# leodd/Lifted-Hybrid-Variational-Inference

Hardware: AMD Instinct MI355X
Metric: lbp_sweeps_per_sec_10M_edge_hybrid_mrf (higher is better)
Workload: dtype f64

## Files before the change

include/lhvi.h:

```cpp
#ifndef LHVI_H
#define LHVI_H

#include <stddef.h>
#include <stdint.h>

#ifdef __cplusplus
extern "C" {
#endif

#define LHVI_ABI_VERSION 19
#define LHVI_MAX_ARITY 6

#define LHVI_OK 0
#define LHVI_E_ARG (-1)
#define LHVI_E_LAUNCH (-2)
#define LHVI_E_UNSUPPORTED (-3)
#define LHVI_E_NODEVICE (-4)
#define LHVI_E_NOT_PD (-5)

#define LHVI_POT_GENERIC 0
#define LHVI_POT_TABLE 1
#define LHVI_POT_GAUSSIAN 2
#define LHVI_POT_QUADRATIC 3
#define LHVI_POT_HYBRID_QUADRATIC 4
#define LHVI_POT_LINEAR_GAUSSIAN 5
#define LHVI_POT_X2 6
#define LHVI_POT_XY 7
#define LHVI_POT_MLN 8
#define LHVI_POT_MLN_HARD 9
#define LHVI_POT_IMAGE_NODE 10
#define LHVI_POT_IMAGE_EDGE 11

typedef struct lhvi_graph {
// ... 68 lines not shown
int lhvi_log_likelihood(const lhvi_graph_t* g, const lhvi_pots_t* pots, const double* x, double* out, void* ws, size_t ws_bytes,
                        void* stream);


#define LHVI_PBP_EP 1u
#define LHVI_PBP_EPBP_DISCRETE 2u
#define LHVI_PBP_SKIP_TERMS 16u
#define LHVI_PBP_LEAVE_ROOM 256u
#define LHVI_PBP_CQ 512u
#define LHVI_PBP_BOUNDARY_TOTALS 2048u
#define LHVI_PBP_NO_UNIQ 4096u
#define LHVI_PBP_V2F_RECORDS 8192u
#define LHVI_PBP_WIDE_PAIRS 16384u
#define LHVI_PBP_SHARE_CUS 32768u
#define LHVI_PBP_NO_GRID 128u
#define LHVI_PBP_FUSED_RECORDS16 131072u
#define LHVI_PBP_F2V_HEAVY 262144u
#define LHVI_PBP_F2V_SMALL 524288u
#define LHVI_PBP_F2V_PAIR 1048576u
#define LHVI_PBP_F2V_FAST 2097152u
#define LHVI_PBP_F2V_CQ 4194304u
#define LHVI_PBP_F2V_GENERIC 8388608u
#define LHVI_PBP_F2V_ALL (LHVI_PBP_F2V_HEAVY | LHVI_PBP_F2V_SMALL | LHVI_PBP_F2V_PAIR | LHVI_PBP_F2V_FAST | LHVI_PBP_F2V_CQ | LHVI_PBP_F2V_GENERIC)
#define LHVI_PBP_POW2_GROUPS 65536u

typedef struct lhvi_pbp {
    int32_t n;
    int32_t T;
    uint32_t flags;
    double var_threshold;
    double max_log_value;
    const double* particles;
    const double* old_particles;
    const int32_t* np;
    const uint8_t* uniq;
    const double* q;
    const int32_t* fast_edges;
    int32_t n_fast;
    const int32_t* generic_edges;
    int32_t n_generic;
    int32_t generic_pts_log2;
    const void* fast_desc;
    const void* heavy_desc;
    int32_t n_heavy;
    const void* light_desc;
    int32_t n_light;
// ... 13 lines not shown
    const void* cq_desc;
    int32_t n_cq;
    const int32_t* v2f_wide;
    int32_t n_v2f_wide;
    const int32_t* v2f_narrow;
    int32_t n_v2f_narrow;
    const int32_t* v2f_hub;
    int32_t n_v2f_hub;
    const int32_t* v2f_mid16;
    int32_t n_v2f_mid16;
    const int32_t* v2f_mid32;
    int32_t n_v2f_mid32;
    const int32_t* prop_hub;
    int32_t n_prop_hub;
    double* prop_partial;
    const int32_t* resample_vars;
    int32_t n_resample_vars;
    const void* small16_desc;
    int32_t n_small16;
    const void* small32_desc;
    int32_t n_small32;
    const int64_t* halo_off;
    double* halo_buf;
} lhvi_pbp_t;

#define LHVI_PBP_DESC_BYTES 128
#define LHVI_PBP_TICKET_WORDS 16
#define LHVI_PBP_TICKET_COUNTERS 8
int lhvi_pbp_describe(const lhvi_graph_t* g, const lhvi_pots_t* pots, const lhvi_pbp_t* s, const int32_t* edges, int32_t count,
                      void* desc_out, void* stream);
int lhvi_pbp_describe_cq(const lhvi_graph_t* g, const lhvi_pots_t* pots, const lhvi_pbp_t* s, const int32_t* edges, int32_t count,
                         void* desc_out, void* stream);
int lhvi_pbp_var_sum(const lhvi_graph_t* g, const lhvi_pbp_t* s, const double* f2v, double* out, void* stream);
int lhvi_pbp_domain_grid(const lhvi_graph_t* g, const lhvi_pbp_t* s, double* x, void* stream);
int lhvi_pbp_refine_grid(const lhvi_graph_t* g, const lhvi_pbp_t* s, const double* logb, double* x, double* best, double* best_val,
                         void* stream);
int lhvi_debug_exp(const double* x, double* y, int64_t n, void* stream);
int lhvi_debug_exp_acc(const double* x, const double* c, double* y, int64_t n, void* stream);
int lhvi_debug_exp_acc_floor(const double* x, const double* c, double* y, int64_t n, void* stream);
int lhvi_debug_log(const double* x, double* y, int64_t n, int32_t which, void* stream);

int lhvi_pbp_classify(const lhvi_graph_t* g, const lhvi_pots_t* pots, const lhvi_pbp_t* s, uint8_t* edge_class, void* stream);

int lhvi_pbp_uniq(const lhvi_graph_t* g, int32_t n, const double* particles, const int32_t* np, uint8_t* uniq, void* stream);
int lhvi_pbp_v2f(const lhvi_graph_t* g, const lhvi_pbp_t* s, const double* f2v, double* v2f, void* stream);
int lhvi_pbp_f2v(const lhvi_graph_t* g, const lhvi_pots_t* pots, const lhvi_pbp_t* s, const double* v2f, double* f2v, void* stream);
int lhvi_pbp_proposal(const lhvi_graph_t* g, const lhvi_pbp_t* s, const double* f2v, double* eta, double* q, void* stream);
int lhvi_pbp_proposal_partial(const lhvi_graph_t* g, const lhvi_pbp_t* s, const double* f2v, double* eta, double* ph, void* stream);
int lhvi_pbp_proposal_finish(const lhvi_graph_t* g, const lhvi_pbp_t* s, const double* ph, double* q, void* stream);
int lhvi_pbp_boundary_pack(const lhvi_graph_t* g, const lhvi_pbp_t* s, const double* f2v, const double* ph, int32_t nb,
                           const int32_t* bvars, double* send, void* stream);
int lhvi_pbp_boundary_reduce(int32_t n_items, const int32_t* width, const int32_t* src_ptr, const int64_t* src_off,
                             const int32_t* dst_ptr, const int64_t* dst_off, const double* in, double* out, void* stream);
int lhvi_pbp_init(const lhvi_graph_t* g, const lhvi_pbp_t* s, double* eta, double* q, double* f2v, double* v2f, void* stream);
int lhvi_pbp_resample(const lhvi_graph_t* g, const lhvi_pbp_t* s, const int64_t* var_gid, uint64_t seed, uint32_t iteration, double* particles_out, void* stream);
int lhvi_pbp_edge_points(const lhvi_graph_t* g, const lhvi_pots_t* pots, const lhvi_pbp_t* s, const double* v2f,
                         int32_t nq, const int32_t* qedge, int32_t npts, const double* x, double* out, void* stream);
int lhvi_pbp_resample_uniq(const lhvi_graph_t* g, const lhvi_pbp_t* s, const int64_t* var_gid, uint64_t seed, uint32_t iteration,
                           double* particles_out, uint8_t* uniq_out, void* stream);
int lhvi_pbp_belief_points(const lhvi_graph_t* g, const lhvi_pots_t* pots, const lhvi_pbp_t* s, const double* v2f,
                           int32_t nq, const int32_t* qvar, int32_t npts, const double* x, double* out, void* stream);
int lhvi_pbp_var_fused(const lhvi_graph_t* g, const lhvi_pbp_t* s, const double* f2v, double* v2f, double* eta, double* q,
                       const int64_t* var_gid, uint64_t seed, uint32_t iteration, double* particles_out, uint8_t* uniq_out,
                       const int32_t* desc, int32_t n16, int32_t n32_t32, int32_t n32_t64, void* stream);
int lhvi_pbp_quad(const lhvi_graph_t* g, const lhvi_pots_t* pots, const lhvi_pbp_t* s, const double* v2f, int64_t nq,
                  const int32_t* row_var, const int64_t* qptr, const int32_t* qedge, const double* qmult, const double* lo,
                  const double* hi, double epsabs, double epsrel, double* z, double* abserr, int32_t* status, void* stream);
int lhvi_pbp_map_brent(const lhvi_graph_t* g, const lhvi_pots_t* pots, const lhvi_pbp_t* s, const double* v2f, int64_t nq,
// ... 235 lines not shown
```

lifted-hybrid-variational-inference_amd/csrc/pbp.hip:

```cpp
#include "common.hpp"
#include "potential.hpp"
#include "fastmath.hpp"
#include "cq.hpp"

namespace lhvi {

__device__ __forceinline__ double wave_sum(double v) { return dpp_wave_reduce(v, SumOp()); }
__device__ __forceinline__ double wave_max(double v) { return dpp_wave_reduce(v, MaxOp()); }
__device__ __forceinline__ int wave_sum_i(int v) {
#pragma unroll
    for (int off = 32; off > 0; off >>= 1) v += __shfl_xor(v, off);
    return v;
}

constexpr double PAD_LOG_TERM = -6.0e5;

__host__ __device__ __forceinline__ int var_first(const lhvi_pbp_t& s) { return s.var_hi > s.var_lo ? s.var_lo : 0; }
__host__ __device__ __forceinline__ int var_limit(const lhvi_graph_t& g, const lhvi_pbp_t& s) { return s.var_hi > s.var_lo ? s.var_hi : g.V; }

__device__ __forceinline__ double norm_pdf_std(double x, double mu, double sig) {
    const double u = (x - mu) / sig;
    return exp(-u * u * 0.5) / (2.506628274631 * sig);
}

__device__ __forceinline__ double log_importance(const lhvi_graph_t& g, const lhvi_pbp_t& s, int v, int d, double x,
                                                 double mu, double rsd , double log_norm) {
    const double LOG_1E200 = 460.51701859880916;
    if (g.dom_cont[d]) {
        if (x == g.dom_lo[d] || x == g.dom_hi[d]) return -LOG_1E200;
    } else {
        if (!(s.flags & LHVI_PBP_EPBP_DISCRETE)) return 0.0;
        const int b = g.dom_ptr[d];
        const int ns = g.dom_ptr[d + 1] - b;
        if (x == g.dom_val[b] || (ns > 1 && x == g.dom_val[b + 1])) return -LOG_1E200;
    }
    const double u = (x - mu) * rsd;
    return fmin(u * u * 0.5 + log_norm, LOG_1E200);
}

__global__ void __launch_bounds__(BLOCK) pbp_uniq_kernel(int V, int n, const double* __restrict__ particles,
                                                        const int32_t* __restrict__ np, uint8_t* __restrict__ uniq) {
    const int64_t i = (int64_t)blockIdx.x * BLOCK + threadIdx.x;
    if (i >= (int64_t)V * n) return;
    const int v = (int)(i / n), j = (int)(i % n);
    int u = j < np[v];
    const double x = particles[i];
    const double* row = particles + (int64_t)v * n;
    for (int k = 0; k < j && u; ++k)
// ... 884 lines not shown
    auto p = (const __attribute__((address_space(4))) char*)__builtin_amdgcn_kernarg_segment_ptr();
    asm volatile("" : "+s"(p));
    return *(const __attribute__((address_space(4))) T*)(p + offset);
}
struct HeavyHead {
    int32_t e, tv, pv, pce, cls, pos, kind, nj, np, T, gb, par_off;
    double pval;
    int32_t type, grid;
};
struct HeavyCoef { double ay, by, c, axy, bx, kx, gx0, gh; };
struct HeavyDesc { HeavyHead h; HeavyCoef k; };
static_assert(sizeof(HeavyDesc) == sizeof(FastDesc) && offsetof(HeavyDesc, k) == offsetof(FastDesc, ay) &&
              offsetof(HeavyHead, pval) == offsetof(FastDesc, pval) && offsetof(HeavyHead, grid) == offsetof(FastDesc, pad) + 4 &&
              offsetof(HeavyCoef, gx0) + offsetof(HeavyDesc, k) == offsetof(FastDesc, pad2), "HeavyDesc is FastDesc in two halves");

template <typename T> using global_ptr = __attribute__((address_space(1))) T*;
template <typename T>
__device__ __forceinline__ global_ptr<T> scalar_row(T* p) { global_ptr<T> q = (global_ptr<T>)p; asm("" : "+s"(q)); return q; }

template <typename T>
__device__ __forceinline__ T row_load(global_ptr<T> row, uint32_t i) { return *(global_ptr<T>)((global_ptr<const char>)row + i * (uint32_t)sizeof(T)); }
template <typename T>
__device__ __forceinline__ void row_store(global_ptr<T> row, uint32_t i, T v) { *(global_ptr<T>)((global_ptr<char>)row + i * (uint32_t)sizeof(T)) = v; }

__device__ __forceinline__ HeavyData heavy_fetch(const HeavyHead& d, const HeavyArgs& s, const double* __restrict__ v2f, int lane) {
    HeavyData h;
    const int n = s.n, np = d.np, npts = grid_eligible(d.grid, d.nj, d.T) ? d.np : d.np + d.T;
    const uint32_t ul = (uint32_t)lane;
    const auto prow = scalar_row(s.particles + (int64_t)d.tv * n);
    const auto grid_row = [&] { return scalar_row(heavy_arg_reload<const double*>(offsetof(HeavyArgs, dom_val)) + d.gb); };
    h.y = d.pval; h.m = 0.0; h.x0 = 0.0; h.x1 = 0.0;
    if (is_hidden(d.pval) && lane < d.nj) {
        h.y = row_load(scalar_row(s.old_particles + (int64_t)d.pv * n), ul);
        h.m = row_load(scalar_row(v2f + (int64_t)d.pce * n), ul);
    }
    if (np == 64 && npts == 64) {
        h.x0 = row_load(prow, ul);
    } else {
        const int pl = lane & ((1 << round_log2_width(npts)) - 1);
        if (pl < npts) h.x0 = pl < np ? row_load(prow, (uint32_t)pl) : row_load(grid_row(), (uint32_t)(pl - np));
    }
    if (npts > 64) {
        const int rem = npts - 64, pl = lane & ((1 << round_log2_width(rem)) - 1), pp = 64 + pl;
        if (pl < rem) h.x1 = pp < np ? row_load(prow, (uint32_t)pp) : row_load(grid_row(), (uint32_t)(pp - np));
    }
    return h;
// ... 1696 lines not shown
        out[(int64_t)v * n + j] = x;
    }
    int u = valid;
    for (int k = 0; k + 1 < W; ++k) {
        const double xk = __shfl(x, first_lane + k);
        if (k < j && k < np && xk == x) u = 0;
    }
    if (on && j < n) uniq[(int64_t)v * n + j] = (uint8_t)u;
}

static int validate_pbp(const lhvi_graph_t* g, const lhvi_pbp_t* s) {
    if (!g || !s) return LHVI_E_ARG;
    if (g->V < 0 || g->E < 0 || s->n <= 0 || s->T < 0) return LHVI_E_ARG;
    if (g->V > 0 && (!g->var_ptr || !g->var_edge || !g->var_value || !g->var_dom || !g->dom_cont || !g->dom_ptr ||
                     !s->particles || !s->np)) return LHVI_E_ARG;
    if (s->var_hi > s->var_lo ? (s->var_lo < 0 || s->var_hi > g->V) : (s->var_lo != 0 || s->var_hi != 0)) return LHVI_E_ARG;
    return LHVI_OK;
}

}

using namespace lhvi;

template <bool HALO>
static int launch_v2f(const lhvi_graph_t* g, const lhvi_pbp_t* s, const double* f2v, double* v2f, void* stream) {
    if (s->v2f_wide || s->v2f_narrow) {
        if (!s->v2f_wide || !s->v2f_narrow || s->n_v2f_wide < 0 || s->n_v2f_narrow < 0 || s->bslot || s->var_hi > s->var_lo) return LHVI_E_ARG;
        if (s->n_v2f_wide > 0)
            hipLaunchKernelGGL(pbp_v2f_kernel<HALO>, dim3(grid_for((int64_t)s->n_v2f_wide * WAVE)), dim3(BLOCK), 0, as_stream(stream), *g, *s, f2v, v2f);
        if (s->v2f_hub && s->n_v2f_hub > 0)
            hipLaunchKernelGGL(pbp_v2f_hub_kernel<HALO>, dim3((unsigned)s->n_v2f_hub), dim3(BLOCK), 0, as_stream(stream), *g, *s, f2v, v2f);
        if (s->n_v2f_narrow > 0)
            hipLaunchKernelGGL(pbp_v2f_narrow_kernel<HALO>, dim3(grid_for(((int64_t)s->n_v2f_narrow + 15) / 16 * WAVE)), dim3(BLOCK), 0,
                               as_stream(stream), *g, *s, f2v, v2f);
        if (s->n_v2f_mid16 < 0 || s->n_v2f_mid32 < 0 || (s->n_v2f_mid16 > 0 && !s->v2f_mid16) || (s->n_v2f_mid32 > 0 && !s->v2f_mid32)) return LHVI_E_ARG;
        if (s->n_v2f_mid16 > 0)
            hipLaunchKernelGGL((pbp_v2f_packed_kernel<16, HALO>), dim3(grid_for(((int64_t)s->n_v2f_mid16 + 3) / 4 * WAVE)), dim3(BLOCK), 0,
                               as_stream(stream), *g, *s, f2v, v2f, s->v2f_mid16, s->n_v2f_mid16);
        if (s->n_v2f_mid32 > 0)
            hipLaunchKernelGGL((pbp_v2f_packed_kernel<32, HALO>), dim3(grid_for(((int64_t)s->n_v2f_mid32 + 1) / 2 * WAVE)), dim3(BLOCK), 0,
                               as_stream(stream), *g, *s, f2v, v2f, s->v2f_mid32, s->n_v2f_mid32);
        return check_launch();
    }
    hipLaunchKernelGGL(pbp_v2f_kernel<HALO>, dim3(grid_for((int64_t)(var_limit(*g, *s) - var_first(*s)) * WAVE)), dim3(BLOCK), 0, as_stream(stream),
                       *g, *s, f2v, v2f);
    return check_launch();
}

template <int W>
static void launch_f2v_pair_small(const lhvi_graph_t* g, const lhvi_pbp_t* s, const double* v2f, double* f2v, int cus, int spare, void* stream) {
    static const int per_cu = blocks_per_cu((const void*)pbp_f2v_pair_small_kernel<W>);
// ... 70 lines not shown
    return check_launch();
}

int lhvi_debug_exp_acc_floor(const double* x, const double* c, double* y, int64_t n, void* stream) {
    if (n < 0 || (n > 0 && (!x || !c || !y))) return LHVI_E_ARG;
    if (n == 0) return LHVI_OK;
    hipLaunchKernelGGL(debug_exp_acc_floor_kernel, dim3(grid_for(n)), dim3(BLOCK), 0, as_stream(stream), x, c, y, n);
    return check_launch();
}

int lhvi_debug_exp_acc(const double* x, const double* c, double* y, int64_t n, void* stream) {
    if (!x || !c || !y || n < 0) return LHVI_E_ARG;
    if (n == 0) return LHVI_OK;
    hipLaunchKernelGGL(debug_exp_acc_kernel, dim3(grid_for(n)), dim3(BLOCK), 0, as_stream(stream), x, c, y, n);
    return check_launch();
}

int lhvi_pbp_v2f(const lhvi_graph_t* g, const lhvi_pbp_t* s, const double* f2v, double* v2f, void* stream) {
    if (int rc = validate_pbp(g, s)) return rc;
    if (!f2v || !v2f || !s->uniq || !s->q) return LHVI_E_ARG;
    if (s->halo_off && !s->halo_buf) return LHVI_E_ARG;
    if (g->V == 0) return LHVI_OK;
    return s->halo_off ? launch_v2f<true>(g, s, f2v, v2f, stream) : launch_v2f<false>(g, s, f2v, v2f, stream);
}

int lhvi_pbp_f2v(const lhvi_graph_t* g, const lhvi_pots_t* pots, const lhvi_pbp_t* s, const double* v2f, double* f2v, void* stream) {
    if (int rc = validate_pbp(g, s)) return rc;
    if (!pots || !v2f || !f2v || !s->old_particles) return LHVI_E_ARG;
    if ((s->flags & LHVI_PBP_CQ) && (!s->fast_edges || !s->generic_edges)) return LHVI_E_ARG;
    if (s->n_small16 < 0 || s->n_small32 < 0 || (s->n_small16 > 0 && !s->small16_desc) || (s->n_small32 > 0 && !s->small32_desc)) return LHVI_E_ARG;
    if (g->E == 0) return LHVI_OK;
    const int nfast = s->fast_edges ? s->n_fast : g->E, ngen = s->generic_edges ? s->n_generic : g->E;
    static const int cus = device_cus();
    static const int fast_per_cu = blocks_per_cu((const void*)pbp_f2v_fast_kernel);
    static const int heavy_per_cu = blocks_per_cu((const void*)pbp_f2v_heavy_kernel, HEAVY_BLOCK);
    static const int light_per_cu = blocks_per_cu((const void*)pbp_f2v_light_kernel);
    static const int gen_per_cu = blocks_per_cu((const void*)pbp_f2v_generic_kernel<true>);
    static const int gen_slim_per_cu = blocks_per_cu((const void*)pbp_f2v_generic_kernel<false>);
    const int share = (s->flags & LHVI_PBP_SHARE_CUS) ? 1 : 0;
    const int spare = (s->flags & LHVI_PBP_LEAVE_ROOM) ? max(cus / 8, 1) : 0;
    auto short_grid = [&](int items, int per_cu) { return dim3(min((items + 3) / 4, max(cus * min(per_cu, 8) - spare, 1))); };
    const uint32_t families = s->flags & LHVI_PBP_F2V_ALL;
    auto want = [families](uint32_t family) { return families == 0 || (families & family) != 0; };
    if (want(LHVI_PBP_F2V_HEAVY) && s->heavy_desc && s->n_heavy > 0) {
        constexpr int HWPB = HEAVY_BLOCK / WAVE;
        const int heavy_grid = min((s->n_heavy + HWPB - 1) / HWPB, max(cus * max(heavy_per_cu - share, 1) - spare * (BLOCK / WAVE) / HWPB, 1));
// ... 284 lines not shown
```

lifted-hybrid-variational-inference_amd/lhvi/_abi.py:

```python
from __future__ import annotations

import ctypes as C
import os

import numpy as np

_HERE = os.path.dirname(os.path.abspath(__file__))
LIB_PATH = os.environ.get('LHVI_LIB') or os.path.join(os.path.dirname(_HERE), 'csrc', 'liblhvi.so')

c_i32p = C.c_void_p
c_f64p = C.c_void_p


class LhviError(RuntimeError):
    pass


class GraphStruct(C.Structure):
    _fields_ = [
        ('V', C.c_int32), ('F', C.c_int32), ('E', C.c_int32), ('nnz', C.c_int32),
        ('fac_ptr', C.c_void_p), ('edge_var', C.c_void_p), ('edge_fac', C.c_void_p), ('edge_canon', C.c_void_p),
        ('var_ptr', C.c_void_p), ('var_edge', C.c_void_p), ('edge_count', C.c_void_p), ('fac_pot', C.c_void_p),
        ('var_value', C.c_void_p), ('var_dom', C.c_void_p), ('var_mult', C.c_void_p), ('fac_mult', C.c_void_p),
        ('D', C.c_int32),
# ... 13 lines not shown

class PbpStruct(C.Structure):
    _fields_ = [
        ('n', C.c_int32), ('T', C.c_int32), ('flags', C.c_uint32),
        ('var_threshold', C.c_double), ('max_log_value', C.c_double),
        ('particles', C.c_void_p), ('old_particles', C.c_void_p), ('np', C.c_void_p), ('uniq', C.c_void_p),
        ('q', C.c_void_p),
        ('fast_edges', C.c_void_p), ('n_fast', C.c_int32), ('generic_edges', C.c_void_p), ('n_generic', C.c_int32),
        ('generic_pts_log2', C.c_int32), ('fast_desc', C.c_void_p), ('heavy_desc', C.c_void_p), ('n_heavy', C.c_int32), ('light_desc', C.c_void_p), ('n_light', C.c_int32),
        ('bslot', C.c_void_p), ('brow_ptr', C.c_void_p), ('brow_off', C.c_void_p), ('brow_peer', C.c_void_p),
        ('recv', C.c_void_p), ('rank', C.c_int32), ('var_degree', C.c_void_p),
        ('var_lo', C.c_int32), ('var_hi', C.c_int32),
        ('f2v_ticket', C.c_void_p),
        ('prop_desc', C.c_void_p), ('n_prop_desc', C.c_int32),
        ('pair_desc', C.c_void_p), ('n_pair', C.c_int32),
        ('cq_desc', C.c_void_p), ('n_cq', C.c_int32),
        ('v2f_wide', C.c_void_p), ('n_v2f_wide', C.c_int32), ('v2f_narrow', C.c_void_p), ('n_v2f_narrow', C.c_int32),
        ('v2f_hub', C.c_void_p), ('n_v2f_hub', C.c_int32),
        ('v2f_mid16', C.c_void_p), ('n_v2f_mid16', C.c_int32), ('v2f_mid32', C.c_void_p), ('n_v2f_mid32', C.c_int32),
        ('prop_hub', C.c_void_p), ('n_prop_hub', C.c_int32), ('prop_partial', C.c_void_p),
        ('resample_vars', C.c_void_p), ('n_resample_vars', C.c_int32),
        ('small16_desc', C.c_void_p), ('n_small16', C.c_int32), ('small32_desc', C.c_void_p), ('n_small32', C.c_int32),
        ('halo_off', C.c_void_p), ('halo_buf', C.c_void_p),
    ]


class ViStruct(C.Structure):
    _fields_ = [
        ('K', C.c_int32), ('T', C.c_int32), ('Dmax', C.c_int32), ('quirks', C.c_int32),
        ('gh_x', C.c_void_p), ('gh_w', C.c_void_p), ('w', C.c_void_p), ('eta_c', C.c_void_p), ('eta_d', C.c_void_p),
        ('obs_var', C.c_void_p), ('var_N', C.c_void_p),
        ('fac_list', C.c_void_p), ('n_cc', C.c_int32), ('n_grp3', C.c_int32), ('n_grp6', C.c_int32), ('n_rest3', C.c_int32),
        ('n_rest6', C.c_int32), ('n_tiny', C.c_int32), ('tiny_par_words', C.c_int32), ('edge_axis', C.c_void_p),
    ]


class ViOptStruct(C.Structure):
    _fields_ = [(n, C.c_void_p) for n in ('w_tau', 'w', 'eta_c', 'tau_d', 'eta_d', 'm_w', 's_w', 'm_c', 's_c', 'm_d', 's_d',
                                          'g_w', 'g_c', 'g_d', 'fe')] + \
               [(n, C.c_double) for n in ('lr', 'b1', 'b2', 'eps', 'var_min')] + [('t', C.c_int32)]


PBP_EP = 1
PBP_EPBP_DISCRETE = 2
PBP_SKIP_TERMS = 16
PBP_NO_GRID = 128
PBP_LEAVE_ROOM = 256
PBP_BOUNDARY_TOTALS = 2048
PBP_CQ = 512
PBP_NO_UNIQ = 4096
PBP_V2F_RECORDS = 8192
PBP_WIDE_PAIRS = 16384
PBP_SHARE_CUS = 32768
PBP_POW2_GROUPS = 65536
PBP_FUSED_RECORDS16 = 131072
PBP_F2V_HEAVY = 262144
PBP_F2V_SMALL = 524288
PBP_F2V_PAIR = 1048576
PBP_F2V_FAST = 2097152
PBP_F2V_CQ = 4194304
PBP_F2V_GENERIC = 8388608
PBP_F2V_ALL = PBP_F2V_HEAVY | PBP_F2V_SMALL | PBP_F2V_PAIR | PBP_F2V_FAST | PBP_F2V_CQ | PBP_F2V_GENERIC
ABI_VERSION = 19
PBP_DESC_BYTES = 128
COLOR_HASH, COLOR_SORT = 0, 1
HUB_DEGREE = 64
VI_GROUP_SLOTS, VI_GROUP_COMP, VI_TINY_NODES, VI_TINY_K, VI_TINY_PAR = 24, 48, 32, 2, 3072

class MwsStruct(C.Structure):
    _fields_ = [('T', C.c_int32), ('max_flips', C.c_int32), ('epsilon', C.c_double), ('noise_std', C.c_double),
                ('seed', C.c_uint64), ('try_id', C.c_void_p), ('disc', C.c_void_p), ('n_disc', C.c_int32),
                ('num', C.c_void_p), ('n_num', C.c_int32), ('fac_class', C.c_void_p), ('x', C.c_void_p), ('best_x', C.c_void_p),
                ('cur_score', C.c_void_p), ('best_score', C.c_void_p), ('status', C.c_void_p), ('err_flip', C.c_void_p),
                ('rec_score', C.c_void_p), ('rec_zero', C.c_void_p), ('rec_ticks', C.c_void_p)] + \
               [(n, C.c_void_p) for n in ('rp_init', 'rp_clause', 'rp_walk', 'rp_walk_k', 'rp_noise', 'rp_post', 'out_score',
                                          'out_unsat', 'out_winner', 'out_accept', 'out_val')]


class ExactStruct(C.Structure):
    _fields_ = [('Nd', C.c_int32), ('Nc', C.c_int32), ('M', C.c_int64), ('dstates', C.c_void_p), ('dstride', C.c_void_p),
                ('n_quad', C.c_int32), ('quad_ptr', C.c_void_p), ('quad_desc', C.c_void_p), ('quad_par', C.c_void_p),
                ('n_tab', C.c_int32), ('tab_ptr', C.c_void_p), ('tab_desc', C.c_void_p), ('tab_par', C.c_void_p)]


class GibbsStruct(C.Structure):
    _fields_ = [('ex', ExactStruct), ('dstate_off', C.c_void_p), ('vt_ptr', C.c_void_p), ('vt_fac', C.c_void_p),
# ... 33 lines not shown
    'lhvi_gabp_f2v': (C.c_int, [_G, _P, _vp, _vp, _vp]),
    'lhvi_gabp_run': (C.c_int, [_G, _P, _vp, _vp, C.c_int, _vp]),
    'lhvi_gabp_marginals': (C.c_int, [_G, _vp, _vp, _vp]),
    'lhvi_gabp_pull_workspace_bytes': (C.c_size_t, [_G]),
    'lhvi_gabp_pull': (C.c_int, [_G, _P, _GP, _vp, _vp, C.c_int, _vp]),
    'lhvi_gabp_run_pull': (C.c_int, [_G, _P, _GP, _vp, _vp, C.c_int, _vp, C.c_size_t, _vp]),
    'lhvi_gabp_graph_create': (C.c_int, [_G, _P, _GP, _vp, _vp, _vp, C.c_int, _vp, C.c_size_t, C.POINTER(C.c_void_p)]),
    'lhvi_gabp_graph_launch': (C.c_int, [_vp, _vp]),
    'lhvi_gabp_graph_destroy': (C.c_int, [_vp]),
    'lhvi_pbp_uniq': (C.c_int, [_G, _i32, _vp, _vp, _vp, _vp]),
    'lhvi_pbp_classify': (C.c_int, [_G, _P, _S, _vp, _vp]),
    'lhvi_pbp_describe': (C.c_int, [_G, _P, _S, _vp, _i32, _vp, _vp]),
    'lhvi_pbp_describe_cq': (C.c_int, [_G, _P, _S, _vp, _i32, _vp, _vp]),
    'lhvi_log_likelihood_workspace_bytes': (C.c_size_t, [_G]),
    'lhvi_log_likelihood': (C.c_int, [_G, _P, _vp, _vp, _vp, C.c_size_t, _vp]),
    'lhvi_pbp_var_sum': (C.c_int, [_G, _S, _vp, _vp, _vp]),
    'lhvi_pbp_domain_grid': (C.c_int, [_G, _S, _vp, _vp]),
    'lhvi_pbp_refine_grid': (C.c_int, [_G, _S, _vp, _vp, _vp, _vp, _vp]),
    'lhvi_debug_exp': (C.c_int, [_vp, _vp, _i64, _vp]),
    'lhvi_debug_log': (C.c_int, [_vp, _vp, _i64, C.c_int32, _vp]),
    'lhvi_debug_exp_acc': (C.c_int, [_vp, _vp, _vp, _i64, _vp]),
    'lhvi_debug_exp_acc_floor': (C.c_int, [_vp, _vp, _vp, _i64, _vp]),
    'lhvi_pbp_v2f': (C.c_int, [_G, _S, _vp, _vp, _vp]),
    'lhvi_pbp_f2v': (C.c_int, [_G, _P, _S, _vp, _vp, _vp]),
    'lhvi_pbp_proposal': (C.c_int, [_G, _S, _vp, _vp, _vp, _vp]),
    'lhvi_pbp_proposal_partial': (C.c_int, [_G, _S, _vp, _vp, _vp, _vp]),
    'lhvi_pbp_proposal_finish': (C.c_int, [_G, _S, _vp, _vp, _vp]),
    'lhvi_pbp_boundary_pack': (C.c_int, [_G, _S, _vp, _vp, _i32, _vp, _vp, _vp]),
    'lhvi_pbp_boundary_reduce': (C.c_int, [_i32, _vp, _vp, _vp, _vp, _vp, _vp, _vp, _vp]),
    'lhvi_pbp_halo_pack': (C.c_int, [_vp, _i32, _i32, _vp, _vp, _vp, _vp, _i32, _vp, _vp, _vp, _vp]),
    'lhvi_pbp_halo_unpack': (C.c_int, [_vp, _i32, _i32, _vp, _vp, _vp, _vp, _i32, _vp, _vp, _vp, _vp]),
    'lhvi_pbp_init': (C.c_int, [_G, _S, _vp, _vp, _vp, _vp, _vp]),
    'lhvi_pbp_resample': (C.c_int, [_G, _S, _vp, _u64, _u32, _vp, _vp]),
    'lhvi_pbp_edge_points': (C.c_int, [_G, _P, _S, _vp, _i32, _vp, _i32, _vp, _vp, _vp]),
    'lhvi_pbp_resample_uniq': (C.c_int, [_G, _S, _vp, _u64, _u32, _vp, _vp, _vp]),
    'lhvi_pbp_belief_points': (C.c_int, [_G, _P, _S, _vp, _i32, _vp, _i32, _vp, _vp, _vp]),
    'lhvi_pbp_map_brent': (C.c_int, [_G, _P, _S, _vp, _i64, _vp, _vp, _vp, _vp, _f64, _i32, _vp, _vp, _vp, _vp]),
    'lhvi_pbp_var_fused': (C.c_int, [_G, _S, _vp, _vp, _vp, _vp, _vp, _u64, _u32, _vp, _vp, _vp, _i32, _i32, _i32, _vp]),
    'lhvi_pbp_quad': (C.c_int, [_G, _P, _S, _vp, _i64, _vp, _vp, _vp, _vp, _vp, _vp, _f64, _f64, _vp, _vp, _vp, _vp]),
    'lhvi_vi_workspace_bytes': (_sz, [_G, _VI]),
    'lhvi_vi_grad': (C.c_int, [_G, _P, _VI, _vp, _vp, _vp, _vp, _vp, _sz, _vp]),
    'lhvi_vi_adam_run': (C.c_int, [_G, _P, _VI, C.POINTER(ViOptStruct), _i32, _vp, _vp, _sz, _vp]),
    'lhvi_adam_step': (C.c_int, [_vp, _vp, _vp, _vp, _i64, _i32, _f64, _f64, _f64, _f64, _i32, _f64, _vp]),
    'lhvi_softmax_rows': (C.c_int, [_vp, _vp, _i64, _i32, _i32, _vp]),
    'lhvi_vi_map_bfgs': (C.c_int, [_G, _VI, _i64, _vp, _f64, _i32, _vp, _vp, _vp, _vp, _vp]),
    'lhvi_color_workspace_bytes': (_sz, [_G]),
# ... 232 lines not shown
```

lifted-hybrid-variational-inference_amd/lhvi/pbp.py:

```python
from __future__ import annotations

import os
from math import e, log, sqrt

import numpy as np

from . import _abi
from .flat import flatten

_F2V_LONG = _abi.PBP_F2V_HEAVY | _abi.PBP_F2V_SMALL
_F2V_SHORT = _abi.PBP_F2V_PAIR | _abi.PBP_F2V_FAST | _abi.PBP_F2V_CQ | _abi.PBP_F2V_GENERIC
F2V_SCHEDULES = {
    'one': (('main', _abi.PBP_F2V_ALL, 0, False),),
    'timed': (('main', _F2V_LONG, 0, True), ('main', _F2V_SHORT, 0, False)),
    'overlap': (('side', _F2V_SHORT, 0, False), ('main', _F2V_LONG, _abi.PBP_SHARE_CUS, True)),
}


class _ParticleSweep:
    var_threshold = 3
    max_log_value = 700
    _epbp_discrete = True
    verbose = False
    listed_proposal = True
# ... 17 lines not shown
        flat = flat if flat is not None else flatten(graph_like, require_device_potentials=True)
        self.flat = flat
        self.dg = dg = _abi.DeviceGraph(flat)
        torch = _abi.require_gpu()
        n = self.n
        sizes = np.diff(flat.dom_ptr)
        cont = flat.dom_cont.astype(bool)
        self.T = int(sizes[cont].max()) if cont.any() else 0
        nst = flat.var_nstates
        if (flat.var_hidden & ~flat.var_cont & (nst > n)).any():
            raise _abi.LhviError('a discrete variable has more states than particle slots n=%d' % n)
        if (flat.var_hidden & flat.var_cont & (np.diff(flat.var_ptr) == 0)).any():
            raise ZeroDivisionError('a hidden continuous variable has no incident factor: its proposal is an empty product')
        self.np_host = np.where(flat.var_hidden, np.where(flat.var_cont, n, nst), 0).astype(np.int32)
        host_lists = {'np_dev': self.np_host}
        S = n + self.T
        self.f2v = dg.zeros(flat.E, S)
        self.v2f = dg.zeros(flat.E, n)
        self.eta = dg.zeros(flat.E, 2)
        self.q_dev = dg.zeros(flat.V, 2)
        self.particles = dg.zeros(flat.V, n)
        self.old_particles = dg.zeros(flat.V, n)
        self.uniq = torch.zeros(flat.V, n, dtype=torch.uint8, device=dg.device)
        self.f2v_ticket = torch.zeros(16, dtype=torch.int32, device=dg.device)
        self.flags = (_abi.PBP_EP if self.proposal_approximation == 'EP' else 0) | \
                     (_abi.PBP_EPBP_DISCRETE if self._epbp_discrete else 0) | \
                     (_abi.PBP_CQ if self.cq_routing and bool((flat.pot_kind == 8).any()) else 0) | \
                     (_abi.PBP_POW2_GROUPS if os.environ.get('LHVI_PBP_POW2_GROUPS', '0') == '1' else 0)
        self._views, self._batched = {}, {}
        self._draws = 0
        self.cq_desc, self.n_cq = None, 0
        self.fast_edges = self.generic_edges = self._fast_list = self._generic_list = torch.zeros(1, dtype=torch.int32, device=dg.device)
        pv_all = np.flatnonzero(flat.var_hidden & flat.var_cont)
        pv = pv_all if owned is None else pv_all[pv_all < owned]
        pd = np.zeros((pv.size, 8), dtype=np.int32)
        pdeg = np.diff(flat.var_ptr)[pv]
        pdom = flat.var_dom[pv]
        pd[:, 0], pd[:, 1], pd[:, 2], pd[:, 3] = pv, pdeg, flat.dom_ptr[pdom], sizes[pdom]
        pbase = flat.var_ptr[pv].astype(np.int64)
        for k in range(4):
            if flat.var_edge.size:
                pd[:, 4 + k] = flat.var_edge[np.minimum(pbase + np.minimum(k, np.maximum(pdeg - 1, 0)), flat.var_edge.size - 1)]
        rdom = flat.var_dom[pv_all]
        rr = np.zeros((pv_all.size, 8), dtype=np.int32)
        rr[:, 0], rr[:, 1] = pv_all, self.np_host[pv_all]
        rr[:, 2:4] = np.ascontiguousarray(flat.dom_lo[rdom], dtype=np.float64).view(np.int32).reshape(-1, 2)
# ... 67 lines not shown
            rest_parts = []
            if 'v2f_wide' in host_lists:
                for name, m in parts:
                    vs = hidden_v[m]
                    vs = vs[~fused_var[vs]]
                    host_lists['v2f_rest_' + name] = (self._v2f_records(flat, vs) if name == 'wide' and os.environ.get('LHVI_PBP_V2F_REC', '1') != '0' else
                                                      vs.astype(np.int32) if vs.size else np.zeros(1, dtype=np.int32))
                    rest_parts.append((name, int(vs.size)))
            self._fused = dict(counts=(int(k16.sum()), int(k32a.sum()), int(k32b.sum())), n_prop_rest=int(keep.sum()),
                               n_resample_rest=int(rkeep.sum()), rest_parts=rest_parts)
        dev_lists = _abi.upload(host_lists)
        for name in ('np_dev', 'resample_vars', '_static_idx', 'prop_desc'):
            setattr(self, name, dev_lists[name])
        if self._fused is not None:
            F = self._fused
            F['desc'], F['prop_desc_rest'], F['resample_rest'] = dev_lists['fused_desc'], dev_lists['prop_desc_rest'], dev_lists['resample_rest']
            F['v2f_rest'] = tuple(x for name, cnt in F['rest_parts'] for x in (dev_lists['v2f_rest_' + name], cnt)) if F['rest_parts'] else None
        if 'prop_hub' in dev_lists:
            self.prop_hub = dev_lists['prop_hub']
        if 'v2f_wide' in dev_lists:
            self.v2f_lists = tuple(x for name, m in parts for x in (dev_lists['v2f_' + name], int(m.sum())))
            if os.environ.get('LHVI_PBP_V2F_REC', '1') != '0':
                self.flags |= _abi.PBP_V2F_RECORDS
        pad = torch.zeros(1, dtype=torch.int32, device=dg.device)
        self.cq_edges = pad[:0]
        self.part_counts = {'heavy': 0, 'light': 0, 'fast': 0, 'generic': 0, 'cq': 0, 'pair': 0, 'small16': 0, 'small32': 0}
        self.generic_pts_log2 = 6
        self.fast_desc = self.heavy_desc = self.light_desc = self.pair_desc = self.small16_desc = self.small32_desc = None
        self.n_heavy = self.n_light = self.n_pair = self.n_small16 = self.n_small32 = self.n_heavy_class = 0
        self.cq_terms = self.heavy_terms = self.heavy_grid_terms = 0
        self._has_f_side = 'f' in sides
        if not self._has_f_side:
            self.fast_edges = self.generic_edges = pad[:0]
            self._fast_list = self._generic_list = pad
            return
        cls = torch.zeros(max(flat.E, 1), dtype=torch.uint8, device=dg.device)
        _abi.check(_abi.lib().lhvi_pbp_classify(dg.g, dg.p, self._struct(), _abi.ptr(cls), _abi.stream_ptr()))
        cls = cls[:flat.E]
        if edge_skip is not None:
            cls = torch.where(_abi.to_dev(np.ascontiguousarray(edge_skip, dtype=bool)), torch.zeros_like(cls), cls)
        self.fast_edges = torch.nonzero((cls == 1) | (cls == 2)).flatten().to(torch.int32)
        self.generic_edges = torch.nonzero(cls == 3).flatten().to(torch.int32)
        self.cq_edges = torch.nonzero(cls == 4).flatten().to(torch.int32)
        key_dev = None
        if edge_key is not None:
            key_dev = _abi.to_dev(np.ascontiguousarray(edge_key, dtype=np.int32))
# ... 104 lines not shown
        if n2:
            r2, rd = w2[rest], d2[rest]
            ow[n1:, 0], ow[n1:, 1] = -1, r2[:, 0].int()
            ow[n1:, 2], ow[n1:, 3] = r2[:, 2].int(), r2[:, 1].int()
            ow[n1:, 4], ow[n1:, 7] = r2[:, 7].int(), r2[:, 8].int()
            od[n1:, 4], od[n1:, 5] = rd[:, 6], nan
            od[n1:, 6:12] = rd[:, 8:14]
            ow[n1:, 25] = r2[:, 3].int()
        first = 0
        if key_dev is not None and n1 + n2:
            edge = torch.where(ow[:, 0] >= 0, ow[:, 0], ow[:, 1]).long()
            order = torch.sort(key_dev[edge], stable=True).indices
            out = out[order].contiguous()
            first = int((key_dev[edge] == 0).sum().item())
        self.pair_desc, self.n_pair = out, n1 + n2
        self.part_counts['pair'] = first

    def _struct(self):
        s = _abi.PbpStruct()
        s.n, s.T, s.flags = self.n, self.T, self.flags
        s.var_threshold, s.max_log_value = float(self.var_threshold), float(self.max_log_value)
        s.particles, s.old_particles = _abi.ptr(self.particles), _abi.ptr(self.old_particles)
        s.np, s.uniq, s.q = _abi.ptr(self.np_dev), _abi.ptr(self.uniq), _abi.ptr(self.q_dev)
        s.fast_edges, s.n_fast = _abi.ptr(self._fast_list), int(self.fast_edges.numel())
        s.generic_edges, s.n_generic = _abi.ptr(self._generic_list), int(self.generic_edges.numel())
        s.generic_pts_log2 = int(getattr(self, 'generic_pts_log2', 6))
        s.fast_desc = _abi.ptr(getattr(self, 'fast_desc', None))
        s.heavy_desc, s.n_heavy = _abi.ptr(getattr(self, 'heavy_desc', None)), int(getattr(self, 'n_heavy', 0))
        s.light_desc, s.n_light = _abi.ptr(getattr(self, 'light_desc', None)), int(getattr(self, 'n_light', 0))
        if getattr(self, 'n_small16', 0):
            s.small16_desc, s.n_small16 = _abi.ptr(self.small16_desc), int(self.n_small16)
        if getattr(self, 'n_small32', 0):
            s.small32_desc, s.n_small32 = _abi.ptr(self.small32_desc), int(self.n_small32)
        if self.paired_light and getattr(self, 'pair_desc', None) is not None:
            s.pair_desc, s.n_pair = _abi.ptr(self.pair_desc), int(self.n_pair)
        s.cq_desc, s.n_cq = _abi.ptr(getattr(self, 'cq_desc', None)), int(getattr(self, 'n_cq', 0))
        if getattr(self, 'v2f_lists', None) is not None:
            w, nw, nr, nn, hb, nh, m16, n16, m32, n32 = self.v2f_lists
            s.v2f_wide, s.n_v2f_wide, s.v2f_narrow, s.n_v2f_narrow = _abi.ptr(w), nw, _abi.ptr(nr), nn
            s.v2f_hub, s.n_v2f_hub = _abi.ptr(hb), nh
            s.v2f_mid16, s.n_v2f_mid16, s.v2f_mid32, s.n_v2f_mid32 = _abi.ptr(m16), n16, _abi.ptr(m32), n32
        s.f2v_ticket = _abi.ptr(self.f2v_ticket) if self.dynamic_f2v else None
        if self.listed_proposal and getattr(self, 'prop_desc', None) is not None:
            s.prop_desc, s.n_prop_desc = _abi.ptr(self.prop_desc), self.n_prop_desc
            if getattr(self, 'prop_hub', None) is not None:
                s.prop_hub, s.n_prop_hub, s.prop_partial = _abi.ptr(self.prop_hub), self.n_prop_hub, _abi.ptr(self.prop_partial)
# ... 941 lines not shown
```

Baseline: 68.24.

## Add lean record-based v2f kernel with compact args and precomputed proposal constants

Adds a specialized variable-to-factor kernel for wide records that takes a small argument struct instead of the full graph and PBP structs. It forces 8 waves per EU, reloads rarely-used pointers from kernel args, and can read precomputed 1/sd and log-normaliser values from a table filled by a small pre-kernel. The aim is lower register and SGPR pressure for higher occupancy, plus avoiding a per-record sqrt, reciprocal and log. The cost is an extra kernel launch per sweep and a new ABI field. The path is gated by flags and only applies when n <= 64 with no halo or bslot.

```diff
diff --git a/include/lhvi.h b/include/lhvi.h
--- a/include/lhvi.h
+++ b/include/lhvi.h
@@ -8,7 +8,7 @@
 extern "C" {
 #endif
 
-#define LHVI_ABI_VERSION 19
+#define LHVI_ABI_VERSION 20
 #define LHVI_MAX_ARITY 6
 
 #define LHVI_OK 0
@@ -123,6 +123,7 @@
 #define LHVI_PBP_F2V_CQ 4194304u
 #define LHVI_PBP_F2V_GENERIC 8388608u
 #define LHVI_PBP_F2V_ALL (LHVI_PBP_F2V_HEAVY | LHVI_PBP_F2V_SMALL | LHVI_PBP_F2V_PAIR | LHVI_PBP_F2V_FAST | LHVI_PBP_F2V_CQ | LHVI_PBP_F2V_GENERIC)
+#define LHVI_PBP_V2F_LEAN 16777216u
 #define LHVI_PBP_POW2_GROUPS 65536u
 
 typedef struct lhvi_pbp {
@@ -182,6 +183,7 @@
     int32_t n_small32;
     const int64_t* halo_off;
     double* halo_buf;
+    double* q_consts;
 } lhvi_pbp_t;
 
 #define LHVI_PBP_DESC_BYTES 128
@@ -204,6 +206,7 @@
 
 int lhvi_pbp_uniq(const lhvi_graph_t* g, int32_t n, const double* particles, const int32_t* np, uint8_t* uniq, void* stream);
 int lhvi_pbp_v2f(const lhvi_graph_t* g, const lhvi_pbp_t* s, const double* f2v, double* v2f, void* stream);
+int lhvi_pbp_v2f_route(const lhvi_graph_t* g, const lhvi_pbp_t* s);
 int lhvi_pbp_f2v(const lhvi_graph_t* g, const lhvi_pots_t* pots, const lhvi_pbp_t* s, const double* v2f, double* f2v, void* stream);
 int lhvi_pbp_proposal(const lhvi_graph_t* g, const lhvi_pbp_t* s, const double* f2v, double* eta, double* q, void* stream);
 int lhvi_pbp_proposal_partial(const lhvi_graph_t* g, const lhvi_pbp_t* s, const double* f2v, double* eta, double* ph, void* stream);
diff --git a/lifted-hybrid-variational-inference_amd/csrc/pbp.hip b/lifted-hybrid-variational-inference_amd/csrc/pbp.hip
--- a/lifted-hybrid-variational-inference_amd/csrc/pbp.hip
+++ b/lifted-hybrid-variational-inference_amd/csrc/pbp.hip
@@ -23,7 +23,8 @@
     return exp(-u * u * 0.5) / (2.506628274631 * sig);
 }
 
-__device__ __forceinline__ double log_importance(const lhvi_graph_t& g, const lhvi_pbp_t& s, int v, int d, double x,
+template <class G, class S>
+__device__ __forceinline__ double log_importance(const G& g, const S& s, int v, int d, double x,
                                                  double mu, double rsd , double log_norm) {
     const double LOG_1E200 = 460.51701859880916;
     if (g.dom_cont[d]) {
@@ -954,6 +955,103 @@
 __device__ __forceinline__ T row_load(global_ptr<T> row, uint32_t i) { return *(global_ptr<T>)((global_ptr<const char>)row + i * (uint32_t)sizeof(T)); }
 template <typename T>
 __device__ __forceinline__ void row_store(global_ptr<T> row, uint32_t i, T v) { *(global_ptr<T>)((global_ptr<char>)row + i * (uint32_t)sizeof(T)) = v; }
+
+struct V2fArgs {
+    int32_t n, S;
+    uint32_t flags;
+    int32_t n_rec;
+    const int32_t* rec;
+    const double* particles;
+    const uint8_t* uniq;
+    const double* q;
+    const double* q_consts;
+    const int32_t* dom_cont;
+    const double* dom_lo;
+    const double* dom_hi;
+    double max_log_value;
+    const int32_t* var_ptr;
+    const int32_t* var_edge;
+    const int32_t* dom_ptr;
+    const double* dom_val;
+};
+struct V2fDomain {
+    template <typename T> struct Loaded { T value; __device__ __forceinline__ T operator[](int) const { return value; } };
+    Loaded<int32_t> dom_cont;
+    Loaded<double> dom_lo, dom_hi;
+    struct Ptr { __device__ __forceinline__ int operator[](int i) const { return heavy_arg_reload<const int32_t*>(offsetof(V2fArgs, dom_ptr))[i]; } } dom_ptr;
+    struct Val { __device__ __forceinline__ double operator[](int i) const { return heavy_arg_reload<const double*>(offsetof(V2fArgs, dom_val))[i]; } } dom_val;
+};
+
+__global__ void __launch_bounds__(BLOCK) pbp_q_consts_kernel(int n_rec, const int32_t* __restrict__ rec, const double* __restrict__ q,
+                                                            double* __restrict__ out) {
+    const int i = blockIdx.x * BLOCK + threadIdx.x;
+    if (i >= n_rec) return;
+    const int v = rec[8 * (int64_t)i];
+    const double sd = sqrt_pos(q[2 * v + 1]), rsd = rcp_newton(sd);
+    const double log_norm = log_pos(2.506628274631 * sd);
+    st2(out, i, rsd, log_norm);
+}
+
+template <bool TABLE>
+__global__ void __launch_bounds__(BLOCK) __attribute__((amdgpu_waves_per_eu(8, 8))) pbp_v2f_rec_kernel(V2fArgs a, const double* __restrict__ f2v,
+                                                                                                   double* __restrict__ v2f) {
+    const uint32_t lane0 = threadIdx.x & 63;
+    const auto lane_at = [&] { uint32_t l = lane0; asm volatile("" : "+v"(l)); return l; };
+    const int item = __builtin_amdgcn_readfirstlane(blockIdx.x * (BLOCK / WAVE) + (threadIdx.x >> 6));
+    if (item >= a.n_rec) return;
+    const int32_t* rec = a.rec + 8 * (int64_t)item;
+    const int v = rec[0], deg = rec[1], np = rec[2], d = rec[3];
+    const int e4[V2F_CACHE] = {rec[4], rec[5], rec[6], rec[7]};
+    if (np <= 0) return;
+    const V2fDomain dom = {{a.dom_cont[d]}, {a.dom_lo[d]}, {a.dom_hi[d]}, {}, {}};
+    const int n = a.n, S = a.S;
+    const double mu = a.q[2 * v];
+    double rsd, log_norm;
+    if (TABLE) {
+        rsd = a.q_consts[2 * (int64_t)item]; log_norm = a.q_consts[2 * (int64_t)item + 1];
+    } else {
+        const double sd = sqrt_pos(a.q[2 * v + 1]);
+        rsd = rcp_newton(sd);
+        log_norm = log_pos(2.506628274631 * sd);
+    }
+    const bool valid = lane0 < (uint32_t)np;
+    double row[V2F_CACHE];
+#pragma unroll
+    for (int k = 0; k < V2F_CACHE; ++k) row[k] = (k < deg && valid) ? row_load(scalar_row(f2v + (int64_t)e4[k] * S), lane_at()) : 0.0;
+    const double x = valid ? row_load(scalar_row(a.particles + (int64_t)v * n), lane_at()) : 0.0;
+    const bool uq = valid && row_load(scalar_row(a.uniq + (int64_t)v * n), lane_at());
+    double total = 0.0;
+#pragma unroll
+    for (int k = 0; k < V2F_CACHE; ++k)
+        if (k < deg) total += row[k];
+    const auto tail_edge = [&](int k) {
+        const int lo = __builtin_amdgcn_readfirstlane(heavy_arg_reload<const int32_t*>(offsetof(V2fArgs, var_ptr))[v]);
+        return __builtin_amdgcn_readfirstlane(heavy_arg_reload<const int32_t*>(offsetof(V2fArgs, var_edge))[lo + k]);
+    };
+    for (int k = V2F_CACHE; k < deg; ++k) {
+        const double m = valid ? row_load(scalar_row(f2v + (int64_t)tail_edge(k) * S), lane_at()) : 0.0;
+        total += m;
+    }
+    const double logw = valid ? log_importance(dom, a, v, d, x, mu, rsd, log_norm) : 0.0;
+    const int cnt1 = __builtin_popcountll(__ballot(uq));
+    const double rcnt = rcp_newton((double)cnt1);
+    auto emit = [&](int e, double m) {
+        const double res = (total - m) + logw;
+        const double tot = wave_sum(uq ? res : 0.0);
+        const double mean = tot * rcnt;
+        double shift = mean;
+        if (__ballot(uq && (res - mean > a.max_log_value)))
+            shift = wave_max(uq ? res : -__builtin_huge_val()) - a.max_log_value;
+        if (valid) row_store(scalar_row(v2f + (int64_t)e * n), lane_at(), res - shift);
+    };
+#pragma unroll
+    for (int k = 0; k < V2F_CACHE; ++k)
+        if (k < deg) emit(e4[k], row[k]);
+    for (int k = V2F_CACHE; k < deg; ++k) {
+        const int e = tail_edge(k);
+        emit(e, valid ? row_load(scalar_row(f2v + (int64_t)e * S), lane_at()) : 0.0);
+    }
+}
 
 __device__ __forceinline__ HeavyData heavy_fetch(const HeavyHead& d, const HeavyArgs& s, const double* __restrict__ v2f, int lane) {
     HeavyData h;
@@ -2696,11 +2794,34 @@
 
 using namespace lhvi;
 
+static bool v2f_wide_is_lean(const lhvi_graph_t* g, const lhvi_pbp_t* s) {
+    return s->v2f_wide && (s->flags & LHVI_PBP_V2F_RECORDS) && (s->flags & LHVI_PBP_V2F_LEAN) && !g->edge_count && !s->bslot && !s->halo_off &&
+           s->n <= WAVE;
+}
+
+static void launch_v2f_rec(const lhvi_graph_t* g, const lhvi_pbp_t* s, const double* f2v, double* v2f, void* stream) {
+    V2fArgs a;
+    a.n = s->n; a.S = s->n + s->T; a.flags = s->flags & LHVI_PBP_EPBP_DISCRETE; a.n_rec = s->n_v2f_wide;
+    a.rec = s->v2f_wide; a.particles = s->particles; a.uniq = s->uniq; a.q = s->q; a.q_consts = s->q_consts;
+    a.dom_cont = g->dom_cont; a.dom_lo = g->dom_lo; a.dom_hi = g->dom_hi; a.max_log_value = s->max_log_value;
+    a.var_ptr = g->var_ptr; a.var_edge = g->var_edge; a.dom_ptr = g->dom_ptr; a.dom_val = g->dom_val;
+    const dim3 grid(grid_for((int64_t)s->n_v2f_wide * WAVE));
+    if (s->q_consts) {
+        hipLaunchKernelGGL(pbp_q_consts_kernel, dim3(grid_for(s->n_v2f_wide)), dim3(BLOCK), 0, as_stream(stream), s->n_v2f_wide, s->v2f_wide, s->q,
+                           s->q_consts);
+        hipLaunchKernelGGL(pbp_v2f_rec_kernel<true>, grid, dim3(BLOCK), 0, as_stream(stream), a, f2v, v2f);
+    } else {
+        hipLaunchKernelGGL(pbp_v2f_rec_kernel<false>, grid, dim3(BLOCK), 0, as_stream(stream), a, f2v, v2f);
+    }
+}
+
 template <bool HALO>
 static int launch_v2f(const lhvi_graph_t* g, const lhvi_pbp_t* s, const double* f2v, double* v2f, void* stream) {
     if (s->v2f_wide || s->v2f_narrow) {
         if (!s->v2f_wide || !s->v2f_narrow || s->n_v2f_wide < 0 || s->n_v2f_narrow < 0 || s->bslot || s->var_hi > s->var_lo) return LHVI_E_ARG;
-        if (s->n_v2f_wide > 0)
+        if (s->n_v2f_wide > 0 && v2f_wide_is_lean(g, s))
+            launch_v2f_rec(g, s, f2v, v2f, stream);
+        else if (s->n_v2f_wide > 0)
             hipLaunchKernelGGL(pbp_v2f_kernel<HALO>, dim3(grid_for((int64_t)s->n_v2f_wide * WAVE)), dim3(BLOCK), 0, as_stream(stream), *g, *s, f2v, v2f);
         if (s->v2f_hub && s->n_v2f_hub > 0)
             hipLaunchKernelGGL(pbp_v2f_hub_kernel<HALO>, dim3((unsigned)s->n_v2f_hub), dim3(BLOCK), 0, as_stream(stream), *g, *s, f2v, v2f);
@@ -2817,6 +2938,11 @@
     if (s->halo_off && !s->halo_buf) return LHVI_E_ARG;
     if (g->V == 0) return LHVI_OK;
     return s->halo_off ? launch_v2f<true>(g, s, f2v, v2f, stream) : launch_v2f<false>(g, s, f2v, v2f, stream);
+}
+
+int lhvi_pbp_v2f_route(const lhvi_graph_t* g, const lhvi_pbp_t* s) {
+    if (!g || !s) return LHVI_E_ARG;
+    return !v2f_wide_is_lean(g, s) ? 0 : (s->q_consts ? 2 : 1);
 }
 
 int lhvi_pbp_f2v(const lhvi_graph_t* g, const lhvi_pots_t* pots, const lhvi_pbp_t* s, const double* v2f, double* f2v, void* stream) {
diff --git a/lifted-hybrid-variational-inference_amd/lhvi/_abi.py b/lifted-hybrid-variational-inference_amd/lhvi/_abi.py
--- a/lifted-hybrid-variational-inference_amd/lhvi/_abi.py
+++ b/lifted-hybrid-variational-inference_amd/lhvi/_abi.py
@@ -59,6 +59,7 @@
         ('resample_vars', C.c_void_p), ('n_resample_vars', C.c_int32),
         ('small16_desc', C.c_void_p), ('n_small16', C.c_int32), ('small32_desc', C.c_void_p), ('n_small32', C.c_int32),
         ('halo_off', C.c_void_p), ('halo_buf', C.c_void_p),
+        ('q_consts', C.c_void_p),
     ]
 
 
@@ -91,6 +92,7 @@
 PBP_SHARE_CUS = 32768
 PBP_POW2_GROUPS = 65536
 PBP_FUSED_RECORDS16 = 131072
+PBP_V2F_LEAN = 16777216
 PBP_F2V_HEAVY = 262144
 PBP_F2V_SMALL = 524288
 PBP_F2V_PAIR = 1048576
@@ -98,7 +100,7 @@
 PBP_F2V_CQ = 4194304
 PBP_F2V_GENERIC = 8388608
 PBP_F2V_ALL = PBP_F2V_HEAVY | PBP_F2V_SMALL | PBP_F2V_PAIR | PBP_F2V_FAST | PBP_F2V_CQ | PBP_F2V_GENERIC
-ABI_VERSION = 19
+ABI_VERSION = 20
 PBP_DESC_BYTES = 128
 COLOR_HASH, COLOR_SORT = 0, 1
 HUB_DEGREE = 64
@@ -178,6 +180,7 @@
     'lhvi_debug_exp_acc': (C.c_int, [_vp, _vp, _vp, _i64, _vp]),
     'lhvi_debug_exp_acc_floor': (C.c_int, [_vp, _vp, _vp, _i64, _vp]),
     'lhvi_pbp_v2f': (C.c_int, [_G, _S, _vp, _vp, _vp]),
+    'lhvi_pbp_v2f_route': (C.c_int, [_G, _S]),
     'lhvi_pbp_f2v': (C.c_int, [_G, _P, _S, _vp, _vp, _vp]),
     'lhvi_pbp_proposal': (C.c_int, [_G, _S, _vp, _vp, _vp, _vp]),
     'lhvi_pbp_proposal_partial': (C.c_int, [_G, _S, _vp, _vp, _vp, _vp]),
diff --git a/lifted-hybrid-variational-inference_amd/lhvi/pbp.py b/lifted-hybrid-variational-inference_amd/lhvi/pbp.py
--- a/lifted-hybrid-variational-inference_amd/lhvi/pbp.py
+++ b/lifted-hybrid-variational-inference_amd/lhvi/pbp.py
@@ -63,6 +63,7 @@
         self.particles = dg.zeros(flat.V, n)
         self.old_particles = dg.zeros(flat.V, n)
         self.uniq = torch.zeros(flat.V, n, dtype=torch.uint8, device=dg.device)
+        self.q_consts = None
         self.f2v_ticket = torch.zeros(16, dtype=torch.int32, device=dg.device)
         self.flags = (_abi.PBP_EP if self.proposal_approximation == 'EP' else 0) | \
                      (_abi.PBP_EPBP_DISCRETE if self._epbp_discrete else 0) | \
@@ -176,6 +177,10 @@
             self.v2f_lists = tuple(x for name, m in parts for x in (dev_lists['v2f_' + name], int(m.sum())))
             if os.environ.get('LHVI_PBP_V2F_REC', '1') != '0':
                 self.flags |= _abi.PBP_V2F_RECORDS
+                if os.environ.get('LHVI_PBP_V2F_LEAN', '1') != '0':
+                    self.flags |= _abi.PBP_V2F_LEAN
+                    if os.environ.get('LHVI_PBP_V2F_TABLE', '1') != '0':
+                        self.q_consts = dg.zeros(flat.V, 2)
         pad = torch.zeros(1, dtype=torch.int32, device=dg.device)
         self.cq_edges = pad[:0]
         self.part_counts = {'heavy': 0, 'light': 0, 'fast': 0, 'generic': 0, 'cq': 0, 'pair': 0, 'small16': 0, 'small32': 0}
@@ -326,6 +331,7 @@
         s.var_threshold, s.max_log_value = float(self.var_threshold), float(self.max_log_value)
         s.particles, s.old_particles = _abi.ptr(self.particles), _abi.ptr(self.old_particles)
         s.np, s.uniq, s.q = _abi.ptr(self.np_dev), _abi.ptr(self.uniq), _abi.ptr(self.q_dev)
+        s.q_consts = _abi.ptr(getattr(self, 'q_consts', None))
         s.fast_edges, s.n_fast = _abi.ptr(self._fast_list), int(self.fast_edges.numel())
         s.generic_edges, s.n_generic = _abi.ptr(self._generic_list), int(self.generic_edges.numel())
         s.generic_pts_log2 = int(getattr(self, 'generic_pts_log2', 6))
```

Measured after the change: 66.62. -2.4%, worse.
